# zju3dv/Mirror-NeRF

Hardware: AMD Instinct MI355X
Metric: rendered rays/sec (primary+reflected) (higher is better)
Workload: dtype f32 carried as hi/lo f16 pairs (f16 MFMA, f32 accumulate; max |diff| to the fp32 chain 3e-6)

## Files before the change

mirror_nerf_amd/csrc/mnrf_composite.inc:

```
struct CompMaps {
    float* weights;
    float* opacity; float* rgb_map; float* depth; float* mirror_mask;
    float* surf_normal; float* surf_normal_grad; float* normal_dif; float* x_surface;
    const float* rays;
    int white_back;
};

template <class Src>
__device__ __forceinline__ float composite_weight(const Src& src, int S, int s, bool in, int lane, float& carry, float& zv) {
    float alpha = 0.f;
    zv = 0.f;
    if (in) {
        zv = src.z(s);
        const float delta = s + 1 < S ? src.z(s + 1) - zv : 1e10f;
        float sv = src.sigma(s);
        if (src.has_noise()) sv = sv + src.noise(s);
        alpha = 1.f - expf(-delta * fmaxf(sv, 0.f));
    }
    const float t = in ? (1.f - alpha) + 1e-10f : 1.f;
    float incl = t;
#pragma unroll
    for (int o = 1; o < 64; o <<= 1) {
        const float up = __shfl_up(incl, o);
        if (lane >= o) incl *= up;
    }
    float excl = __shfl_up(incl, 1);
    if (lane == 0) excl = 1.f;
    const float w = alpha * (carry * excl);
    carry = carry * __shfl(incl, 63);
    return w;
}

template <class Src>
__device__ __forceinline__ float composite_mirror_value(const Src& src, int S, int lane, float* w_keep) {
    float carry = 1.f;
    float a_m = 0.f;
#pragma unroll
    for (int base = 0; base < S; base += 64) {
        const int s = base + lane;
        const bool in = s < S;
        float zv;
        const float w = composite_weight(src, S, s, in, lane, carry, zv);
        if (in) {
            if (w_keep) w_keep[s] = w;
            a_m += w * src.mirror(s);
        }
    }
    return wave_sum(a_m);
}

template <class Src>
__device__ __forceinline__ void composite_ray(const Src& src, int S, int lane, long long ray, const CompMaps& A) {
    float carry = 1.f;
    float a_op = 0.f, a_d = 0.f, a_m = 0.f, a_nd = 0.f;
    float a_c[3] = {0.f, 0.f, 0.f}, a_n[3] = {0.f, 0.f, 0.f}, a_g[3] = {0.f, 0.f, 0.f};
    for (int base = 0; base < S; base += 64) {
        const int s = base + lane;
        const bool in = s < S;
        float zv, w;
        if (src.has_w()) {
            zv = in ? src.z(s) : 0.f;
            w = in ? src.w(s) : 0.f;
        } else {
            w = composite_weight(src, S, s, in, lane, carry, zv);
        }
        if (in) {
            if (A.weights) A.weights[s] = w;
            a_op += w;
            a_d += w * zv;
            if (src.has_rgb()) { a_c[0] += w * src.rgb(s, 0); a_c[1] += w * src.rgb(s, 1); a_c[2] += w * src.rgb(s, 2); }
            if (src.has_mirror()) a_m += w * src.mirror(s);
            float pn[3] = {0.f, 0.f, 0.f}, gn[3] = {0.f, 0.f, 0.f};
            if (src.has_pn()) {
#pragma unroll
                for (int k = 0; k < 3; ++k) { pn[k] = src.pn(s, k); a_n[k] += pn[k] * w; }
            }
            if (src.has_gn()) {
#pragma unroll
                for (int k = 0; k < 3; ++k) { gn[k] = src.gn(s, k); a_g[k] += gn[k] * w; }
            }
            if (src.has_pn() && src.has_gn()) {
                const float d0 = gn[0] - pn[0], d1 = gn[1] - pn[1], d2 = gn[2] - pn[2];
                a_nd += w * (d0 * d0 + d1 * d1 + d2 * d2);
            }
        }
    }
    a_op = wave_sum(a_op);
    a_d = wave_sum(a_d);
    if (src.has_mirror()) a_m = wave_sum(a_m);
    if (src.has_pn() && src.has_gn()) a_nd = wave_sum(a_nd);
#pragma unroll
    for (int k = 0; k < 3; ++k) {
        if (src.has_rgb()) a_c[k] = wave_sum(a_c[k]);
        if (src.has_pn()) a_n[k] = wave_sum(a_n[k]);
        if (src.has_gn()) a_g[k] = wave_sum(a_g[k]);
    }
    if (lane == 0) {
        if (A.opacity) A.opacity[ray] = a_op;
        if (A.rgb_map) {
#pragma unroll
            for (int k = 0; k < 3; ++k) A.rgb_map[ray * 3 + k] = A.white_back ? a_c[k] + (1.f - a_op) : a_c[k];
        }
        if (A.depth) A.depth[ray] = a_d;
        if (A.mirror_mask) A.mirror_mask[ray] = a_m;
        if (A.surf_normal) { for (int k = 0; k < 3; ++k) A.surf_normal[ray * 3 + k] = a_n[k]; }
        if (A.surf_normal_grad) { for (int k = 0; k < 3; ++k) A.surf_normal_grad[ray * 3 + k] = a_g[k]; }
        if (A.normal_dif) A.normal_dif[ray] = a_nd;
        if (A.x_surface) {
            const float* r = A.rays + ray * 8;
            for (int k = 0; k < 3; ++k) A.x_surface[ray * 3 + k] = r[k] + r[3 + k] * a_d;
        }
    }
}
```

mirror_nerf_amd/csrc/mnrf_field_split.inc:

```
constexpr int CHUNK_BYTES = CHUNK_PAIRS * PAIR_BYTES;
constexpr int WAVES = 4;
constexpr int WG_THREADS = 64 * WAVES;
constexpr int WG_SAMPLES = WAVES * S * 16;
constexpr int PIECES = CHUNK_BYTES / TILE_BYTES / WAVES;
constexpr int U = 2;
constexpr int PF = S == 3 ? 2 : 4;
constexpr int NBUF = PF + U;
typedef unsigned u32x4 __attribute__((ext_vector_type(4)));
typedef unsigned u32x2 __attribute__((ext_vector_type(2)));
typedef _Float16 h2v __attribute__((ext_vector_type(2)));
struct StoreCtx {
    __amdgpu_buffer_rsrc_t rsrc;
    __amdgpu_buffer_rsrc_t rsrc_lo;
    char* base;
    int lane;
    int soff;
    h2v fac[S];
};
__device__ __forceinline__ __amdgpu_buffer_rsrc_t plane_rsrc(char* sample_block) {
    return __builtin_amdgcn_make_buffer_rsrc(sample_block, 0, 0x7fffffff, 0x00020000);
}
static_assert(CHUNK_PAIRS / U == PIECES, "one LDS-DMA piece per wave per unit");
constexpr int LDS_RING = RING_SLOTS * CHUNK_BYTES;
constexpr int LDS_BIAS = LDS_RING;
constexpr int LDS_MASK = LDS_BIAS + BIAS_FLOATS * 4;
constexpr int LDS_PARK = LDS_MASK;
constexpr int HEAD_PARK = 6;
constexpr int LDS_PARK_BYTES = S == 3 ? HEAD_PARK * S * WG_THREADS * 16 : 0;
static_assert(S != 3 || HEAD_PARK * S >= 2 * S * 2, "the encoding operands fit the same region");
constexpr int LDS_TILEQ = LDS_MASK + LDS_PARK_BYTES;
constexpr int LDS_BYTES = LDS_TILEQ + 16;
constexpr int LDS_BYTES_GRAD = LDS_MASK + 8 * S * WG_THREADS * 8;
static_assert(LDS_BYTES_GRAD <= 160 * 1024, "LDS budget");
constexpr int LDS_FUSE = LDS_BYTES;
constexpr int LDS_BYTES_FUSE = LDS_BYTES + 10 * WG_SAMPLES * 4;
static_assert(LDS_BYTES_FUSE <= 160 * 1024, "LDS budget");

#include "mnrf_field_split_common.inc"

__device__ __forceinline__ float wave_sum(float v) {
#pragma unroll
    for (int o = 32; o > 0; o >>= 1) v += __shfl_xor(v, o);
    return v;
}
#include "mnrf_composite.inc"
struct CompLdsSrc {
    const float* f;
    bool pn_on, mir_on;
    __device__ __forceinline__ bool has_w() const { return false; }
    __device__ __forceinline__ float w(int) const { return 0.f; }
    __device__ __forceinline__ bool has_noise() const { return false; }
    __device__ __forceinline__ bool has_rgb() const { return true; }
    __device__ __forceinline__ bool has_mirror() const { return mir_on; }
    __device__ __forceinline__ bool has_pn() const { return pn_on; }
    __device__ __forceinline__ bool has_gn() const { return false; }
    __device__ __forceinline__ float z(int s) const { return f[8 * WG_SAMPLES + s]; }
    __device__ __forceinline__ float sigma(int s) const { return f[s]; }
    __device__ __forceinline__ float noise(int) const { return 0.f; }
    __device__ __forceinline__ float rgb(int s, int k) const { return f[(1 + k) * WG_SAMPLES + s]; }
    __device__ __forceinline__ float mirror(int s) const { return f[7 * WG_SAMPLES + s]; }
    __device__ __forceinline__ float pn(int s, int k) const { return f[(4 + k) * WG_SAMPLES + s]; }
    __device__ __forceinline__ float gn(int, int) const { return 0.f; }
};
struct CompLdsSrcBlended : CompLdsSrc {
    bool colour;
    __device__ __forceinline__ bool has_rgb() const { return colour; }
    __device__ __forceinline__ bool has_w() const { return true; }
    __device__ __forceinline__ float w(int s) const { return f[9 * WG_SAMPLES + s]; }
};
struct CompLdsSrcRgbDepth : CompLdsSrc {
    __device__ __forceinline__ bool has_mirror() const { return false; }
    __device__ __forceinline__ bool has_pn() const { return false; }
};

__device__ __forceinline__ unsigned long long enc_out_of_range(const float (&x)[S][3]) {
    bool big = false;
#pragma unroll
    for (int s = 0; s < S; ++s) big |= !(fabsf(x[s][0]) < ENC_RANGE_LIMIT && fabsf(x[s][1]) < ENC_RANGE_LIMIT && fabsf(x[s][2]) < ENC_RANGE_LIMIT);
    return __builtin_amdgcn_ballot_w64(big);
}

template <int N>
__device__ __forceinline__ void split_b(const float (&x)[S][N], u32x4 (&hi)[S][N / 8], u32x4 (&lo)[S][N / 8],
                                        unsigned long long& sat, float limit = F16_MAX) {
    float tmax = 0.f;
#pragma unroll
    for (int s = 0; s < S; ++s)
#pragma unroll
        for (int T = 0; T < N / 8; ++T)
#pragma unroll
            for (int e = 0; e < 4; ++e) {
                unsigned h, l;
                split2(x[s][8 * T + 2 * e], x[s][8 * T + 2 * e + 1], h, l);
                sat_track<false>(tmax, x[s][8 * T + 2 * e], x[s][8 * T + 2 * e + 1]);
                hi[s][T][e] = h;
                lo[s][T][e] = l;
            }
    sat_flush(sat, tmax, limit);
}

__device__ __forceinline__ f32x4 mfma_f16(const u32x4& a, const u32x4& b, const f32x4& c) {
    return __builtin_amdgcn_mfma_f32_16x16x32_f16(__builtin_bit_cast(h8, a), __builtin_bit_cast(h8, b), c, 0, 0, 0);
}

__device__ __forceinline__ float relu_(float x) {
    const int i = __builtin_bit_cast(int, x);
    return __builtin_bit_cast(float, i > 0 ? i : 0);
}

constexpr int NTASKS = 16 * S;
template <int ACT, bool WANT_MASK>
__device__ __forceinline__ void conv_task(int q, const f32x4 (&pacc)[S][8], u32x4 (&oh)[S][8], u32x4 (&ol)[S][8],
                                          int t0, int half, uint64_t (&mk)[S], float& tmax) {
    const int trel = q / (4 * S), s = (q / 4) % S, nb = 2 * trel + ((q >> 1) & 1), rp = q & 1;
    const float a0 = pacc[s][nb][2 * rp], a1 = pacc[s][nb][2 * rp + 1];
    if (WANT_MASK) {
        mk[s] |= (uint64_t)(a0 > 0.f) << (4 * (8 * half + nb) + 2 * rp);
        mk[s] |= (uint64_t)(a1 > 0.f) << (4 * (8 * half + nb) + 2 * rp + 1);
    }
    const float v0 = ACT == 1 ? relu_(a0) : a0, v1 = ACT == 1 ? relu_(a1) : a1;
    unsigned h, l;
    split2(v0, v1, h, l);
    sat_track<ACT == 1>(tmax, v0, v1);
    oh[s][t0 + trel][2 * (nb & 1) + rp] = h;
    ol[s][t0 + trel][2 * (nb & 1) + rp] = l;
}

template <int NT, int NB, int NACC, int NTA, int JOB, bool WANT_MASK, int USTART, int TPU, int POS, int NPARK = 0, int STB = -1,
          int STN = 4, bool SSCALE = false, int JUMP_T = -1, long long JUMP = 0, bool SKIP = false>
__device__ __forceinline__ void gemm_part_impl(f32x4 (&acc)[S][NACC], const u32x4 (&bh)[S][NTA], const u32x4 (&bl)[S][NTA],
                                               Stream& st, int wave, int lane16, const f32x4 (&pacc)[S][8],
                                               u32x4 (&oh)[S][8], u32x4 (&ol)[S][8], int t0, int half, uint64_t (&mk)[S],
                                               const StoreCtx& sc = StoreCtx{}, bool jump_on = true) {
    static_assert(JUMP == 0 || (JUMP_T >= 0 && JUMP_T % U == 0 && JUMP_T < NT * NB && ((POS + JUMP_T) / U) % PIECES == PIECES - 1 && JUMP % CHUNK_BYTES == 0),
                  "the fill pointer jumps between two chunks");
    static_assert(STB < 0 || (S == 2 && NT * NB / U >= 8 * STN && STB + STN <= NTA), "8 store tasks per operand ride on the part's first units");
    static_assert(NT <= NTA, "B operand count");
    static_assert(JOB < 0 || NTASKS % TPU == 0, "tasks per unit");
    static_assert(JOB < 0 || USTART + NTASKS / TPU <= NT * NB / U, "the job fits the part");
    constexpr int NPAIRS = NT * NB;
    static_assert(NPAIRS % U == 0, "pairs come in units");
    const unsigned ring = (unsigned)(size_t)(__attribute__((address_space(3))) char*)smem + (unsigned)lane16;
    u32x4 ah[NBUF], al[NBUF];
    constexpr int START = POS % CHUNK_PAIRS;
    static_assert(POS % U == 0, "parts start on a unit");
    static_assert(NPAIRS >= PF, "a part is at least as long as the read-ahead");
    unsigned base = ring + st.rd_slot * CHUNK_BYTES;
#pragma unroll
    for (int i = 0; i < PF; ++i) {
        ah[i] = st.ch[i];
        al[i] = st.cl[i];
// ... 591 lines not shown
                    const float a0 = acc[s][0][R0], a1 = acc[s][0][R0 + 1], a2 = acc[s][0][R0 + 2];
                    const float inv = 1.f / sqrtf(fmaxf(a0 * a0 + a1 * a1 + a2 * a2, 1.1920928955078125e-07f));
                    float* o = A.pred_normal + (long long)sidx(s) * 3;
                    out_store(o, a0 * inv); out_store(o + 1, a1 * inv); out_store(o + 2, a2 * inv);
                    if (GRAD && A.save_inv)
                        A.save_inv[idx[s]] = (a0 * a0 + a1 * a1 + a2 * a2) > 1.1920928955078125e-07f ? inv : -inv;
                }
        }
    };
    {
        f32x4 acc[S][1];
        init_bias<1>(acc, BIAS_SIG, gq());
        gemm_part<8, 1, 960, HP>(acc, hh, hl, st, wave, lane16);
        if (FUSE) {
            if (gq() == 0) {
#pragma unroll
                for (int s = 0; s < S; ++s) fz[wave * (S * 16) + s * 16 + m15()] = acc[s][0][0];
            }
        } else if (A.sigma && g == 0) {
#pragma unroll
            for (int s = 0; s < S; ++s)
                if (sval(s)) out_store(A.sigma + sidx(s), acc[s][0][0]);
        }
        if constexpr (FOLD && !RGB_DEPTH) put_normal(acc, std::integral_constant<int, 1>{});
    }

    bool colour = true;
    if (!SIGMA_ONLY) {
        if constexpr (!FOLD) {
            u32x4 nh[S][4], nl[S][4];
            {
                f32x4 acc[S][8];
                init_bias<8>(acc, BIAS_NRM1, gq());
                gemm_part<8, 8, 968, HP, ST0>(acc, hh, hl, st, wave, lane16, at_h(7, 0));
                if (keep) save_acc<8, 0>(A.save_x + (long long)SEC_HN * A.B, 128, 0, acc, idx, valid, g, unused_bits);
                acc_to_b<8, 0, false>(nh, nl, acc, 0, tid, st.sat);
                if constexpr (S == 2) { if (pl) store_planes<4, 4>(sc, SEC_HN / 16, nh, nl); }
            }
            f32x4 acc[S][1];
            init_bias<1>(acc, BIAS_NRM2, gq());
            gemm_part<4, 1, 1032>(acc, nh, nl, st, wave, lane16);
            put_normal(acc, std::integral_constant<int, 0>{});
        }
        const auto mirror_head = [&]() {
            u32x4 mh[S][4], ml[S][4];
            {
                f32x4 acc[S][8];
                init_bias<8>(acc, BIAS_MIR1, gq());
                gemm_part<8, 8, BLENDED ? 968 : FOLD ? FOLD_POS_MIR1 : 1036, HP, ST4, 4, false, JT, JUMP_FROM_MIRB>(acc, hh, hl, st, wave, lane16, at_h(7, 4));
                if (keep) {
                    uint64_t bits[S];
                    save_acc<8, 2>(A.save_x + (long long)SEC_HM * A.B, 128, 0, acc, idx, valid, g, bits);
#pragma unroll
                    for (int s = 0; s < S; ++s) gmask[(9 * S + s) * WG_THREADS + tid] = bits[s];
                } else if (GRAD && pl) {
                    store_sign_mask<8>(acc, gmask + (9 * S) * WG_THREADS + tid);
                }
                acc_to_b<8, 2, false>(mh, ml, acc, 0, tid, st.sat);
                if constexpr (S == 2) { if (pl) store_planes<4, 4>(sc, SEC_HM / 16, mh, ml); }
            }
            f32x4 acc[S][1];
            init_bias<1>(acc, BIAS_MIR2, gq());
            gemm_part<4, 1, BLENDED ? 1032 : FOLD ? FOLD_POS_MIR2 : 1100>(acc, mh, ml, st, wave, lane16);
            if (FUSE) {
                if (gq() == 0) {
#pragma unroll
                    for (int s = 0; s < S; ++s) fz[7 * WG_SAMPLES + wave * (S * 16) + s * 16 + m15()] = sigmoidf_(acc[s][0][0]);
                }
            } else if (A.is_mirror && g == 0) {
#pragma unroll
                for (int s = 0; s < S; ++s)
                    if (sval(s)) out_store(A.is_mirror + sidx(s), sigmoidf_(acc[s][0][0]));
            }
        };
        if constexpr (!FOLD) mirror_head();
        if constexpr (BLENDED) {
            mirror_head();
            skip_pairs4<1036>(st, wave, lane16);
            asm volatile("s_waitcnt lgkmcnt(0)" ::: "memory");
            __builtin_amdgcn_s_barrier();
            asm volatile("" ::: "memory");
            int dl;
            asm volatile("v_mbcnt_lo_u32_b32 %0, -1, 0\n\tv_mbcnt_hi_u32_b32 %0, -1, %0" : "=v"(dl));
            const float mv = composite_mirror_value(CompLdsSrc{fz, false, true}, WG_SAMPLES, dl, wave == 0 ? fz + 9 * WG_SAMPLES : nullptr);
            colour = __builtin_amdgcn_readfirstlane((int)(mv < 0.5f)) != 0 || A.fuse == 4;
        }
        const auto view_operands = [&](u32x4 (&vh)[S][1], u32x4 (&vl)[S][1]) {
            float de[S][8];
            const int gv = gq();
            const int spr = opaque_spr();
#pragma unroll
            for (int s = 0; s < S; ++s) {
                const float* dp = A.dir_emb + (long long)(sidx(s) / spr) * A.dir_stride;
#pragma unroll
                for (int t = 0; t < 8; ++t) {
                    const int e = 16 * (t >> 2) + 4 * gv + (t & 3);
                    de[s][t] = e < ENC_DIR ? dp[e] : 0.f;
                }
            }
            if (keep) save_bform<8>(A.save_x + (long long)SEC_DIRE * A.B, 32, de, idx, valid, g);
            split_b<8>(de, vh, vl, st.sat);
            if constexpr (S == 2) { if (pl) store_planes<1, 1>(sc, SEC_DIRE / 16, vh, vl); }
        };
        if (colour) {
            u32x4 dh[S][4], dl[S][4];
            if constexpr (FOLD) {
                u32x4 vh[S][1], vl[S][1];
                view_operands(vh, vl);
                f32x4 acc[S][8];
                init_bias<8>(acc, BIAS_DIR, gq());
                gemm_part<8, 8, BLENDED ? 1040 : FOLD_POS_DIR, HP>(acc, hh, hl, st, wave, lane16);
                gemm_part<1, 8, BLENDED ? 1104 : FOLD_POS_VIEW>(acc, vh, vl, st, wave, lane16);
                acc_to_b<8, 1, false>(dh, dl, acc, 0, tid, st.sat);
            } else {
                u32x4 fh[S][8], fl[S][8];
                {
                    f32x4 acc[S][16];
                    init_bias<16>(acc, BIAS_FIN, gq());
                    gemm_part<8, 16, 1104, HP>(acc, hh, hl, st, wave, lane16);
                    if (keep) save_acc<16, 0>(A.save_x + (long long)SEC_FIN * A.B, 256, 0, acc, idx, valid, g, unused_bits);
                    acc_to_b<16, 0, false>(fh, fl, acc, 0, tid, st.sat);
                    if constexpr (S == 2) { if (pl) store_planes<8, 8>(sc, SEC_FIN / 16, fh, fl); }
                }
                u32x4 vh[S][1], vl[S][1];
                view_operands(vh, vl);
                f32x4 acc[S][8];
                init_bias<8>(acc, BIAS_DIR, gq());
                gemm_part<8, 8, 1232>(acc, fh, fl, st, wave, lane16);
                gemm_part<1, 8, 1296>(acc, vh, vl, st, wave, lane16);
                if (keep) {
                    uint64_t bits[S];
                    save_acc<8, 1>(A.save_x + (long long)SEC_HD * A.B, 128, 0, acc, idx, valid, g, bits);
#pragma unroll
                    for (int s = 0; s < S; ++s) gmask[(8 * S + s) * WG_THREADS + tid] = bits[s];
                } else if (GRAD && pl) {
                    store_sign_mask<8>(acc, gmask + (8 * S) * WG_THREADS + tid);
                }
                acc_to_b<8, 1, false>(dh, dl, acc, 0, tid, st.sat);
                if constexpr (S == 2) { if (pl) store_planes<4, 4>(sc, SEC_HD / 16, dh, dl); }
            }
            f32x4 acc[S][1];
            init_bias<1>(acc, BIAS_RGB, gq());
            gemm_part<4, 1, BLENDED ? 1112 : FOLD ? FOLD_POS_RGB : 1304>(acc, dh, dl, st, wave, lane16);
            if (FUSE) {
                if (gq() == 0) {
#pragma unroll
                    for (int s = 0; s < S; ++s) {
                        const int q = wave * (S * 16) + s * 16 + (int)m15();
                        fz[1 * WG_SAMPLES + q] = sigmoidf_(acc[s][0][0]);
                        fz[2 * WG_SAMPLES + q] = sigmoidf_(acc[s][0][1]);
                        fz[3 * WG_SAMPLES + q] = sigmoidf_(acc[s][0][2]);
                    }
                }
            } else if (A.rgb && g == 0) {
#pragma unroll
                for (int s = 0; s < S; ++s)
                    if (sval(s)) {
                        float* o = A.rgb + (long long)sidx(s) * 3;
                        out_store(o, sigmoidf_(acc[s][0][0]));
                        out_store(o + 1, sigmoidf_(acc[s][0][1]));
                        out_store(o + 2, sigmoidf_(acc[s][0][2]));
                    }
            }
        }
        if constexpr (FOLD && !RGB_DEPTH && !BLENDED) mirror_head();
    }

// ... 12 lines not shown
                    for (int r = 0; r < 4; ++r) gr[s][4 * nb + r] = v[r];
            }
        }
        float genc[S][16];
#pragma unroll
        for (int s = 0; s < S; ++s)
#pragma unroll
            for (int t = 0; t < 16; ++t) genc[s][t] = 0.f;

#pragma unroll 1
        for (int layer = 7; layer >= 0; --layer) {
            u32x4 gh[S][8], gl[S][8];
#pragma unroll
            for (int s = 0; s < S; ++s) {
                const uint64_t mk = ((const uint64_t*)(smem + LDS_MASK))[(layer * S + s) * WG_THREADS + tid];
#pragma unroll
                for (int t = 0; t < 64; ++t) gr[s][t] = ((mk >> t) & 1ull) ? gr[s][t] : 0.f;
            }
            split_b<64>(gr, gh, gl, st.sat);
            if (layer == 4 || layer == 0) {
                f32x4 acc[S][4];
                zero_acc<4>(acc);
                gemm_part<8, 4, 0>(acc, gh, gl, st, wave, lane16);
#pragma unroll
                for (int s = 0; s < S; ++s)
#pragma unroll
                    for (int nb = 0; nb < 4; ++nb)
#pragma unroll
                        for (int r = 0; r < 4; ++r) genc[s][4 * nb + r] += acc[s][nb][r];
            }
            if (layer != 0) {
                f32x4 acc[S][16];
                zero_acc<16>(acc);
                gemm_part<8, 16, 0>(acc, gh, gl, st, wave, lane16);
#pragma unroll
                for (int s = 0; s < S; ++s)
#pragma unroll
                    for (int nb = 0; nb < 16; ++nb)
#pragma unroll
                        for (int r = 0; r < 4; ++r) gr[s][4 * nb + r] = acc[s][nb][r];
            }
        }
        float x[S][3];
        fetch_positions(x);
#pragma unroll
        for (int s = 0; s < S; ++s) {
            float d0 = 0.f, d1 = 0.f, d2 = 0.f;
#pragma unroll
            for (int pp = 0; pp < 8; ++pp) {
                const int P = 8 * g + pp;
                const int f = P / 3;
                const int a = P - 3 * f;
                const float gs = genc[s][2 * pp], gc = genc[s][2 * pp + 1];
                if (P < 30) {
                    const float xa = a == 0 ? x[s][0] : (a == 1 ? x[s][1] : x[s][2]);
                    float sn, cs;
                    fast_sincos(ldexpf(xa, f), sn, cs);
                    const float c = ldexpf(gs * cs - gc * sn, f);
                    d0 += a == 0 ? c : 0.f;
                    d1 += a == 1 ? c : 0.f;
                    d2 += a == 2 ? c : 0.f;
                } else if (P == 30) {
                    d0 += gs;
                    d1 += gc;
                } else {
                    d2 += gs;
                }
            }
            d0 += __shfl_xor(d0, 16); d1 += __shfl_xor(d1, 16); d2 += __shfl_xor(d2, 16);
            d0 += __shfl_xor(d0, 32); d1 += __shfl_xor(d1, 32); d2 += __shfl_xor(d2, 32);
            if (A.normal && g == 0 && valid[s]) {
                const float n0 = -d0, n1 = -d1, n2 = -d2;
                const float sq = n0 * n0 + n1 * n1 + n2 * n2;
                const float inv = 1.f / sqrtf(fmaxf(sq, 1.1920928955078125e-07f));
                float* o = A.normal + (long long)idx[s] * 3;
                o[0] = n0 * inv; o[1] = n1 * inv; o[2] = n2 * inv;
                if (A.save_invj) A.save_invj[idx[s]] = sq > 1.1920928955078125e-07f ? inv : -inv;
            }
        }
    }
    sat_all |= st.sat;
    enc_all |= enc_range;
    if (FUSE) {
        __syncthreads();
        if (wave == 0) {
            const long long ray = tile;
            int cl;
            asm volatile("v_mbcnt_lo_u32_b32 %0, -1, 0\n\tv_mbcnt_hi_u32_b32 %0, -1, %0" : "=v"(cl));
            if constexpr (RGB_DEPTH) {
                const CompMaps out{A.f_weights ? A.f_weights + ray * WG_SAMPLES : nullptr, A.f_opacity, A.f_rgb_map, A.f_depth, nullptr,
                                   nullptr, nullptr, nullptr, A.f_x_surface, A.rays, A.white_back};
                composite_ray(CompLdsSrcRgbDepth{fz, false, false}, WG_SAMPLES, cl, ray, out);
            } else if constexpr (BLENDED) {
                const CompLdsSrcBlended src{{fz, A.f_surf_normal != nullptr, A.f_mirror_mask != nullptr}, colour};
                const CompMaps out{A.f_weights ? A.f_weights + ray * WG_SAMPLES : nullptr, A.f_opacity, colour ? A.f_rgb_map : nullptr, A.f_depth,
                                   A.f_mirror_mask, A.f_surf_normal, nullptr, nullptr, A.f_x_surface, A.rays, A.white_back};
                composite_ray(src, WG_SAMPLES, cl, ray, out);
                if (!colour && A.f_rgb_map && cl < 3) A.f_rgb_map[ray * 3 + cl] = 0.f;
            } else {
                const CompLdsSrc src{fz, A.f_surf_normal != nullptr, A.f_mirror_mask != nullptr};
                const CompMaps out{A.f_weights ? A.f_weights + ray * WG_SAMPLES : nullptr, A.f_opacity, A.f_rgb_map, A.f_depth, A.f_mirror_mask,
                                   A.f_surf_normal, nullptr, nullptr, A.f_x_surface, A.rays, A.white_back};
                composite_ray(src, WG_SAMPLES, cl, ray, out);
            }
        }
    }
    if (!queued) break;
    close_stream();
    __syncthreads();
    tile = __builtin_amdgcn_readfirstlane(((volatile int*)(smem + LDS_TILEQ))[round & 1]);
    ++round;
    if (tile >= A.n_tiles) break;
    }
    guard_report(A.packed, sat_all, enc_all, MNRF_GUARD_IN_FORWARD);
    close_stream();
    int last_lane;
    asm volatile("v_mbcnt_lo_u32_b32 %0, -1, 0\n\tv_mbcnt_hi_u32_b32 %0, -1, %0" : "=v"(last_lane));
    if (queued && wave == 0 && last_lane == 0) {
        if (atomicAdd(A.tile_queue + 1, 1) == (int)gridDim.x - 1) {
            atomicExch(A.tile_queue, 0);
            atomicExch(A.tile_queue + 1, 0);
        }
    }
}

template <bool SIGMA_ONLY, bool GRAD, bool PLANES = false, bool FUSE = false>
__global__ __launch_bounds__(WG_THREADS, MIN_WAVES_PER_SIMD) void field_split_kernel(FieldArgs A) {
    field_split_body<SIGMA_ONLY, GRAD, PLANES, FUSE, false>(A);
}
template <bool ON = true>
__global__ __launch_bounds__(WG_THREADS, MIN_WAVES_PER_SIMD) void field_split_kernel_rgb_depth(FieldArgs A) {
    field_split_body<false, false, false, ON, ON>(A);
}

template <bool ON = true>
__global__ __launch_bounds__(WG_THREADS, MIN_WAVES_PER_SIMD) void field_split_kernel_blended(FieldArgs A) {
    field_split_body<false, false, false, ON, false, ON>(A);
}

template <bool UNUSED = false>
inline int launch(const FieldArgs& A, bool sigma_only, bool grad, hipStream_t s) {
    const long long blocks64 = (A.B + WG_SAMPLES - 1) / WG_SAMPLES;
    if (blocks64 > 0x7fffffff || A.B > 0x7fffffffLL) return -1;
    dim3 grid((unsigned)blocks64);
    const dim3 block(WG_THREADS);
    if (S == 3 && A.tile_queue) {
        if (A.n_tiles != (int)blocks64 || A.resident < 1 || A.resident > A.n_tiles) return -1;
        grid = dim3((unsigned)A.resident);
    }
    if (sigma_only && !grad) hipLaunchKernelGGL((field_split_kernel<true, false>), grid, block, LDS_BYTES, s, A);
    else if (!sigma_only && !grad && S == 3 && A.fuse == 2) {
        if constexpr (S == 3) hipLaunchKernelGGL((field_split_kernel_rgb_depth<>), grid, block, LDS_BYTES_FUSE, s, A);
    } else if (!sigma_only && !grad && S == 3 && A.fuse >= 3) {
        if constexpr (S == 3) hipLaunchKernelGGL((field_split_kernel_blended<>), grid, block, LDS_BYTES_FUSE, s, A);
    } else if (!sigma_only && !grad && S == 3 && A.fuse)
        hipLaunchKernelGGL((field_split_kernel<false, false, false, S == 3>), grid, block, LDS_BYTES_FUSE, s, A);
    else if (!sigma_only && !grad) hipLaunchKernelGGL((field_split_kernel<false, false>), grid, block, LDS_BYTES, s, A);
#ifndef MNRF_SPLIT_NO_GRAD
    else if (sigma_only && grad) hipLaunchKernelGGL((field_split_kernel<true, true>), grid, block, LDS_BYTES_GRAD, s, A);
    else if (S == 2 && A.save_planes) hipLaunchKernelGGL((field_split_kernel<false, true, S == 2>), grid, block, LDS_BYTES_GRAD, s, A);
    else hipLaunchKernelGGL((field_split_kernel<false, true>), grid, block, LDS_BYTES_GRAD, s, A);
#else
    else return -1;
#endif
    return 0;
}
```

mirror_nerf_amd/csrc/mnrf_render.hip:

```cpp
#include <hip/hip_runtime.h>
#include <stdint.h>
#include <stdio.h>
#include <string.h>

#include "../../include/mnrf.h"
#include "mnrf_error.h"
#include "mnrf_fill.h"
#include "mnrf_rays.h"

static thread_local char g_err[512] = "";

int mnrf_fail(int code, const char* msg) {
    snprintf(g_err, sizeof(g_err), "%s", msg);
    return code;
}

int mnrf_check_launch(const char* where) {
    hipError_t e = hipGetLastError();
    if (e != hipSuccess) {
        snprintf(g_err, sizeof(g_err), "%s: %s", where, hipGetErrorString(e));
        return MNRF_ERR_LAUNCH;
    }
    return MNRF_OK;
}

extern "C" const char* mnrf_last_error(void) { return g_err; }
extern "C" int mnrf_version(void) { return 1; }

namespace {

constexpr float EPS32 = 1.1920928955078125e-07f;

__device__ __forceinline__ long long live_rows(long long cap, const int* __restrict__ n_live) {
    if (!n_live) return cap;
    const long long v = *n_live;
    return v < 0 ? 0 : (v < cap ? v : cap);
}

__device__ __forceinline__ float wave_sum(float v) {
#pragma unroll
    for (int o = 32; o > 0; o >>= 1) v += __shfl_xor(v, o);
    return v;
}
#include "mnrf_composite.inc"

__global__ void embed_kernel(const float* __restrict__ x, long long n, int c, int n_freqs, float* __restrict__ out,
                             const int* __restrict__ n_live) {
    const long long i = (long long)blockIdx.x * blockDim.x + threadIdx.x;
    if (i >= live_rows(n, n_live) * c) return;
    const long long row = i / c;
    const int ch = (int)(i % c);
    const int ld = c * (2 * n_freqs + 1);
    const float v = x[i];
    float* o = out + row * ld;
    o[ch] = v;
    for (int f = 0; f < n_freqs; ++f) {
        float s, co;
        sincosf(ldexpf(v, f), &s, &co);
        o[c * (1 + 2 * f) + ch] = s;
        o[c * (2 + 2 * f) + ch] = co;
    }
}

__global__ void sample_coarse_kernel(const float* __restrict__ rays, long long n_rays, const float* __restrict__ z_steps,
                                     int ns, int use_disp, float perturb, const float* __restrict__ prand,
                                     float* __restrict__ z_out, const int* __restrict__ n_live) {
    const long long i = (long long)blockIdx.x * blockDim.x + threadIdx.x;
    if (i >= live_rows(n_rays, n_live) * ns) return;
    const long long r = i / ns;
    const int s = (int)(i % ns);
    const float near = rays[r * 8 + 6], far = rays[r * 8 + 7];
    auto zat = [&](int k) -> float {
        const float t = z_steps[k];
        if (!use_disp) return near * (1.f - t) + far * t;
        return 1.f / (1.f / near * (1.f - t) + 1.f / far * t);
    };
    float z = zat(s);
    if (perturb > 0.f) {
        const float lower = s == 0 ? z : 0.5f * (zat(s - 1) + z);
        const float upper = s == ns - 1 ? z : 0.5f * (z + zat(s + 1));
        z = lower + (upper - lower) * (perturb * prand[i]);
    }
    z_out[i] = z;
}

struct CompArgs {
    const float* rays; long long n_rays; int S;
    const float* sigma; const float* z; const float* noise; const float* rgb; const float* is_mirror;
    const float* pred_normal; const float* normal; int white_back;
    float* weights; float* opacity; float* rgb_map; float* depth; float* mirror_mask;
    float* surf_normal; float* surf_normal_grad; float* normal_dif; float* x_surface;
    const int* n_live;
};

struct CompGlobalSrc {
    const CompArgs& A;
    long long ray;
    __device__ __forceinline__ bool has_w() const { return false; }
    __device__ __forceinline__ float w(int) const { return 0.f; }
    __device__ __forceinline__ bool has_noise() const { return A.noise != nullptr; }
    __device__ __forceinline__ bool has_rgb() const { return A.rgb != nullptr; }
    __device__ __forceinline__ bool has_mirror() const { return A.is_mirror != nullptr; }
    __device__ __forceinline__ bool has_pn() const { return A.pred_normal != nullptr; }
    __device__ __forceinline__ bool has_gn() const { return A.normal != nullptr; }
    __device__ __forceinline__ float z(int s) const { return A.z[ray * A.S + s]; }
    __device__ __forceinline__ float sigma(int s) const { return A.sigma[ray * A.S + s]; }
    __device__ __forceinline__ float noise(int s) const { return A.noise[ray * A.S + s]; }
    __device__ __forceinline__ float rgb(int s, int k) const { return A.rgb[(ray * A.S + s) * 3 + k]; }
    __device__ __forceinline__ float mirror(int s) const { return A.is_mirror[ray * A.S + s]; }
    __device__ __forceinline__ float pn(int s, int k) const { return A.pred_normal[(ray * A.S + s) * 3 + k]; }
    __device__ __forceinline__ float gn(int s, int k) const { return A.normal[(ray * A.S + s) * 3 + k]; }
};

__global__ __launch_bounds__(256) void composite_kernel(CompArgs A) {
    const int lane = threadIdx.x & 63;
    const long long ray = (long long)blockIdx.x * 4 + (threadIdx.x >> 6);
    if (ray >= live_rows(A.n_rays, A.n_live)) return;
    const CompGlobalSrc src{A, ray};
    const CompMaps out{A.weights ? A.weights + ray * A.S : nullptr, A.opacity, A.rgb_map, A.depth, A.mirror_mask, A.surf_normal,
                       A.surf_normal_grad, A.normal_dif, A.x_surface, A.rays, A.white_back};
    composite_ray(src, A.S, lane, ray, out);
}


struct CompBwdArgs {
    const float* rays; long long n_rays; int S;
    const float* sigma; const float* z; const float* noise; const float* rgb; const float* is_mirror;
    const float* pred_normal; const float* normal; int white_back;
    const float* depth;
    const float* g_w; const float* g_op; const float* g_rgb; const float* g_depth; const float* g_mask;
    const float* g_sn; const float* g_sng; const float* g_nd; const float* g_xs;
    float* d_sigma; float* d_rgb; float* d_mirror; float* d_pn; float* d_n; float* d_rays;
    int detach;
    const float* keep_mirror;
    const int* n_live;
};
constexpr int CB_MAXB = 4;

__global__ __launch_bounds__(256) void composite_backward_kernel(CompBwdArgs A) {
    const int lane = threadIdx.x & 63;
    const long long ray = (long long)blockIdx.x * 4 + (threadIdx.x >> 6);
    if (ray >= live_rows(A.n_rays, A.n_live)) return;
    const int S = A.S;
    const float* r8 = A.rays ? A.rays + ray * 8 : nullptr;
    float gop = A.g_op ? A.g_op[ray] : 0.f;
    float gc[3] = {0.f, 0.f, 0.f}, gsn[3] = {0.f, 0.f, 0.f}, gsg[3] = {0.f, 0.f, 0.f}, gxs[3] = {0.f, 0.f, 0.f};
    if (A.g_rgb) { for (int k = 0; k < 3; ++k) gc[k] = A.g_rgb[ray * 3 + k]; }
    if (A.g_sn) { for (int k = 0; k < 3; ++k) gsn[k] = A.g_sn[ray * 3 + k]; }
    if (A.g_sng) { for (int k = 0; k < 3; ++k) gsg[k] = A.g_sng[ray * 3 + k]; }
    if (A.g_xs) { for (int k = 0; k < 3; ++k) gxs[k] = A.g_xs[ray * 3 + k]; }
    float gd = A.g_depth ? A.g_depth[ray] : 0.f;
    const float gm = A.g_mask ? A.g_mask[ray] : 0.f;
    const float gnd = A.g_nd ? A.g_nd[ray] : 0.f;
    const bool w_mask = !(A.detach & MNRF_DETACH_W_MASK) && !(A.keep_mirror && A.keep_mirror[ray] == 0.f);
    const bool w_nrm = !(A.detach & MNRF_DETACH_W_NORMAL);
    const float gm_w = w_mask ? gm : 0.f;
    const float gnd_w = w_nrm ? gnd : 0.f;
    float gsn_w[3], gsg_w[3];
    for (int k = 0; k < 3; ++k) { gsn_w[k] = w_nrm ? gsn[k] : 0.f; gsg_w[k] = w_nrm ? gsg[k] : 0.f; }
    if (A.g_xs && r8) gd += gxs[0] * r8[3] + gxs[1] * r8[4] + gxs[2] * r8[5];
    if (A.white_back) gop -= gc[0] + gc[1] + gc[2];
    if (A.d_rays && lane == 0) {
        float* o = A.d_rays + ray * 8;
        const float dep = A.depth ? A.depth[ray] : 0.f;
        for (int k = 0; k < 3; ++k) { o[k] = gxs[k]; o[3 + k] = gxs[k] * dep; }
        o[6] = 0.f; o[7] = 0.f;
    }
    float Tn[CB_MAXB], Gw[CB_MAXB], Gv[CB_MAXB], tv[CB_MAXB], dads[CB_MAXB];
    float carry = 1.f;
#pragma unroll
    for (int blk = 0; blk < CB_MAXB; ++blk) {
        Tn[blk] = 0.f; Gw[blk] = 0.f; Gv[blk] = 0.f; tv[blk] = 1.f; dads[blk] = 0.f;
        if (blk * 64 >= S) continue;
        const int s = blk * 64 + lane;
        const bool in = s < S;
        const long long i1 = ray * S + s, i3 = i1 * 3;
        float alpha = 0.f, G = 0.f, delta = 0.f, sv = 0.f, ex = 1.f;
        float pn[3] = {0.f, 0.f, 0.f}, gn[3] = {0.f, 0.f, 0.f};
        if (in) {
            const float zv = A.z[i1];
            delta = s + 1 < S ? A.z[i1 + 1] - zv : 1e10f;
            sv = A.sigma[i1];
// ... 983 lines not shown
```

mirror_nerf_amd/recursion.py:

```python
import ctypes
import os
from collections import defaultdict
import weakref
from types import SimpleNamespace

import torch
from torch import nn

from . import _lib
from .mirror_nerf import Embedding, MirrorNeRF
from .dnerf import render_rays_dnerf
from .rendering import render_rays

RAY_FORWARD_OFFSET = 0.1
BLENDED_BREAK_EVEN = 0.37
_MIRROR_FRACTION = weakref.WeakKeyDictionary()
JITTER_RAYS = 262144

PLACE_MIRROR_PRESETS = {
    "plane_x": (
        ("livingroom", dict(position=0.0, normal=(-1.0, 0.0, 0.0), rect=(-1.0, 1.0, -0.5, 0.5))),
        ("washroom", dict(position=-1.0, normal=(1.0, 0.0, 0.0), rect=(-1.0, 1.0, -1.0, 0.75))),
        ("office", dict(position=1.0, normal=(1.0, 0.0, 0.0), rect=(-1.0, 1.0, -1.0, 0.75))),
        (None, dict(position=-1.0, normal=(1.0, 0.0, 0.0), rect=(-1.0, 1.0, -0.5, 0.5))),
    ),
    "plane_y": (
        ("washroom", dict(position=1.3, normal=(0.0, -1.0, 0.0), rect=(-1.0, 1.0, -1.0, 1.0))),
        ("livingroom", dict(position=1.65, normal=(0.0, -1.0, 0.0), rect=(-0.3, 1.5, -0.5, 1.0))),
        ("office", dict(position=0.0, normal=(0.0, -1.0, 0.0), rect=(-1.0, 1.0, -0.5, 0.5))),
        (None, dict(position=1.0, normal=(0.0, -1.0, 0.0), rect=(-1.0, 1.0, -0.5, 0.5))),
    ),
}
SUBSTITUTION_PRESETS = (
    ("office", dict(rotation=None, scale=1.0, translation=(0.0, 1.0, 0.0))),
    ("market", dict(rotation=((0.0, 1.0, 0.0), (-1.0, 0.0, 0.0), (0.0, 0.0, 1.0)), scale=1.0,
                    translation=(0.0, 0.0, 0.0))),
    (None, dict(rotation=None, scale=1.0, translation=(0.0, 0.0, 0.0))),
)
OBJECT_PRESETS = (
    ("livingroom", dict(pose_align=None, scale=2.0, translation=(0.0, 0.0, 0.0))),
    ("washroom", dict(pose_align=None, scale=2.0, translation=(-0.5, -0.5, 0.0))),
    ("office", dict(pose_align=None, scale=2.0, translation=(0.0, 3.0, 0.5))),
    (None, dict(pose_align=None, scale=1.0, translation=(0.0, 0.0, 0.0))),
)


def _preset(table, root_dir):
    for key, value in table:
        if key is None or key in (root_dir or ""):
            return dict(value)
    raise AssertionError("preset tables end with a default entry")


def resolve_new_mirror(args, new_mirror=None):
    if new_mirror is not None:
        nm = dict(new_mirror)
        missing = {"axis", "position", "normal", "rect"} - set(nm)
        if missing:
            raise ValueError(f"new_mirror needs the keys axis, position, normal, rect (missing: {sorted(missing)})")
        if nm["axis"] not in ("x", "y"):
            raise ValueError(f"new_mirror axis must be 'x' or 'y', not {nm['axis']!r}")
        if len(nm["normal"]) != 3 or len(nm["rect"]) != 4:
            raise ValueError("new_mirror normal has 3 entries and rect 4 (u0, u1, w0, w1)")
        return dict(axis=nm["axis"], position=float(nm["position"]), normal=tuple(float(v) for v in nm["normal"]),
                    rect=tuple(float(v) for v in nm["rect"]))
    plane_pos = getattr(args, "plane_pos", "plane_x")
    if plane_pos not in PLACE_MIRROR_PRESETS:
        raise ValueError(f"args.plane_pos must be 'plane_x' or 'plane_y', not {plane_pos!r}")
    p = _preset(PLACE_MIRROR_PRESETS[plane_pos], getattr(args, "root_dir", ""))
    return dict(axis=plane_pos[-1], **p)


def resolve_substitution(args):
    return _preset(SUBSTITUTION_PRESETS, getattr(args, "root_dir", ""))


def resolve_new_object(args, new_object=None):
    if new_object is not None:
        cfg = dict(new_object)
        missing = {"pose_align", "scale", "translation"} - set(cfg)
        if missing:
            raise ValueError(f"new_object needs the keys pose_align, scale, translation (missing: {sorted(missing)})")
    else:
        cfg = _preset(OBJECT_PRESETS, getattr(args, "root_dir", ""))
    if len(cfg["translation"]) != 3:
        raise ValueError("new_object translation has 3 entries")
    scale = float(cfg["scale"])
    if not scale > 0.0:
        raise ValueError(f"new_object scale must be positive, not {cfg['scale']!r}")
    pose, pose_scale0 = None, 1.0
    if cfg["pose_align"] is not None:
        m = torch.as_tensor(cfg["pose_align"], dtype=torch.float32)
        if tuple(m.shape) not in ((3, 4), (4, 4)):
            raise ValueError(f"new_object pose_align must be None, 3x4 or 4x4, not {tuple(m.shape)}")
        pose = tuple(float(v) for v in m[:3, :4].reshape(-1))
        pose_scale0 = float(torch.norm(m[:3, 0]))
        if not pose_scale0 > 0.0:
            raise ValueError("new_object pose_align: the first column of its 3x3 is zero")
# ... 694 lines not shown
```

Measured before the change: 1.985 million.

## Split fused per-ray compositing across all four waves of the workgroup

```diff
diff --git a/mirror_nerf_amd/csrc/mnrf_composite.inc b/mirror_nerf_amd/csrc/mnrf_composite.inc
--- a/mirror_nerf_amd/csrc/mnrf_composite.inc
+++ b/mirror_nerf_amd/csrc/mnrf_composite.inc
@@ -7,8 +7,9 @@
 };
 
 template <class Src>
-__device__ __forceinline__ float composite_weight(const Src& src, int S, int s, bool in, int lane, float& carry, float& zv) {
-    float alpha = 0.f;
+__device__ __forceinline__ void composite_block_scan(const Src& src, int S, int s, bool in, int lane, float& alpha, float& zv, float& excl,
+                                                     float& total) {
+    alpha = 0.f;
     zv = 0.f;
     if (in) {
         zv = src.z(s);
@@ -24,29 +25,18 @@
         const float up = __shfl_up(incl, o);
         if (lane >= o) incl *= up;
     }
-    float excl = __shfl_up(incl, 1);
+    excl = __shfl_up(incl, 1);
     if (lane == 0) excl = 1.f;
+    total = __shfl(incl, 63);
+}
+
+template <class Src>
+__device__ __forceinline__ float composite_weight(const Src& src, int S, int s, bool in, int lane, float& carry, float& zv) {
+    float alpha, excl, total;
+    composite_block_scan(src, S, s, in, lane, alpha, zv, excl, total);
     const float w = alpha * (carry * excl);
-    carry = carry * __shfl(incl, 63);
+    carry = carry * total;
     return w;
-}
-
-template <class Src>
-__device__ __forceinline__ float composite_mirror_value(const Src& src, int S, int lane, float* w_keep) {
-    float carry = 1.f;
-    float a_m = 0.f;
-#pragma unroll
-    for (int base = 0; base < S; base += 64) {
-        const int s = base + lane;
-        const bool in = s < S;
-        float zv;
-        const float w = composite_weight(src, S, s, in, lane, carry, zv);
-        if (in) {
-            if (w_keep) w_keep[s] = w;
-            a_m += w * src.mirror(s);
-        }
-    }
-    return wave_sum(a_m);
 }
 
 template <class Src>
@@ -57,13 +47,8 @@
     for (int base = 0; base < S; base += 64) {
         const int s = base + lane;
         const bool in = s < S;
-        float zv, w;
-        if (src.has_w()) {
-            zv = in ? src.z(s) : 0.f;
-            w = in ? src.w(s) : 0.f;
-        } else {
-            w = composite_weight(src, S, s, in, lane, carry, zv);
-        }
+        float zv;
+        const float w = composite_weight(src, S, s, in, lane, carry, zv);
         if (in) {
             if (A.weights) A.weights[s] = w;
             a_op += w;
@@ -112,3 +97,113 @@
         }
     }
 }
+
+constexpr int COMP_WG_SAMPLES = 192;
+
+__device__ __forceinline__ void composite_wg_barrier() {
+    asm volatile("s_waitcnt lgkmcnt(0)" ::: "memory");
+    __builtin_amdgcn_s_barrier();
+    asm volatile("" ::: "memory");
+}
+
+template <class Src>
+__device__ __forceinline__ void composite_weights_wg(const Src& src, int wave, int lane, float* totals, float* w_row, float* w_out) {
+    const int s = wave * 64 + lane;
+    float alpha = 0.f, zv = 0.f, excl = 1.f, total = 1.f;
+    if (wave < 3) {
+        composite_block_scan(src, COMP_WG_SAMPLES, s, true, lane, alpha, zv, excl, total);
+        if (lane == 0) totals[wave] = total;
+    }
+    composite_wg_barrier();
+    if (wave < 3) {
+        float carry = 1.f;
+        if (wave >= 1) carry = carry * totals[0];
+        if (wave >= 2) carry = carry * totals[1];
+        const float w = alpha * (carry * excl);
+        w_row[s] = w;
+        if (w_out) w_out[s] = w;
+    }
+    composite_wg_barrier();
+}
+
+template <class X>
+__device__ __forceinline__ float composite_wg_sum(const float* w_row, int lane, const X& x) {
+    float a = 0.f;
+#pragma unroll
+    for (int base = 0; base < COMP_WG_SAMPLES; base += 64) a += w_row[base + lane] * x(base + lane);
+    return wave_sum(a);
+}
+__device__ __forceinline__ float composite_wg_opacity(const float* w_row, int lane) {
+    float a = 0.f;
+#pragma unroll
+    for (int base = 0; base < COMP_WG_SAMPLES; base += 64) a += w_row[base + lane];
+    return wave_sum(a);
+}
+
+template <class Src>
+__device__ __forceinline__ void composite_maps_wg(const Src& src, int wave, int lane, const float* w_row, long long ray, const CompMaps& A) {
+    if (A.weights && wave < 3) A.weights[wave * 64 + lane] = w_row[wave * 64 + lane];
+    if (wave == 0) {
+        const float a_op = composite_wg_opacity(w_row, lane);
+        const float a_d = composite_wg_sum(w_row, lane, [&](int s) { return src.z(s); });
+        if (lane == 0) {
+            if (A.opacity) A.opacity[ray] = a_op;
+            if (A.depth) A.depth[ray] = a_d;
+            if (A.x_surface) {
+                const float* r = A.rays + ray * 8;
+                for (int k = 0; k < 3; ++k) A.x_surface[ray * 3 + k] = r[k] + r[3 + k] * a_d;
+            }
+        }
+    } else if (wave == 1) {
+        if (A.rgb_map) {
+            float a_c[3] = {0.f, 0.f, 0.f};
+            if (src.has_rgb()) {
+#pragma unroll
+                for (int k = 0; k < 3; ++k) a_c[k] = composite_wg_sum(w_row, lane, [&](int s) { return src.rgb(s, k); });
+            }
+            float a_op = 0.f;
+            if (A.white_back) a_op = composite_wg_opacity(w_row, lane);
+            if (lane == 0) {
+#pragma unroll
+                for (int k = 0; k < 3; ++k) A.rgb_map[ray * 3 + k] = A.white_back ? a_c[k] + (1.f - a_op) : a_c[k];
+            }
+        }
+    } else if (wave == 2) {
+        if (src.has_pn() || src.has_gn()) {
+            float a_n[3] = {0.f, 0.f, 0.f}, a_g[3] = {0.f, 0.f, 0.f}, a_nd = 0.f;
+#pragma unroll
+            for (int k = 0; k < 3; ++k) {
+                if (src.has_pn()) a_n[k] = composite_wg_sum(w_row, lane, [&](int s) { return src.pn(s, k); });
+                if (src.has_gn()) a_g[k] = composite_wg_sum(w_row, lane, [&](int s) { return src.gn(s, k); });
+            }
+            if (src.has_pn() && src.has_gn())
+                a_nd = composite_wg_sum(w_row, lane, [&](int s) {
+                    const float d0 = src.gn(s, 0) - src.pn(s, 0), d1 = src.gn(s, 1) - src.pn(s, 1), d2 = src.gn(s, 2) - src.pn(s, 2);
+                    return d0 * d0 + d1 * d1 + d2 * d2;
+                });
+            if (lane == 0) {
+                if (A.surf_normal) { for (int k = 0; k < 3; ++k) A.surf_normal[ray * 3 + k] = a_n[k]; }
+                if (A.surf_normal_grad) { for (int k = 0; k < 3; ++k) A.surf_normal_grad[ray * 3 + k] = a_g[k]; }
+                if (A.normal_dif) A.normal_dif[ray] = a_nd;
+            }
+        } else if (lane == 0) {
+            if (A.surf_normal) { for (int k = 0; k < 3; ++k) A.surf_normal[ray * 3 + k] = 0.f; }
+            if (A.surf_normal_grad) { for (int k = 0; k < 3; ++k) A.surf_normal_grad[ray * 3 + k] = 0.f; }
+            if (A.normal_dif) A.normal_dif[ray] = 0.f;
+        }
+    } else {
+        if (A.mirror_mask) {
+            float a_m = 0.f;
+            if (src.has_mirror()) a_m = composite_wg_sum(w_row, lane, [&](int s) { return src.mirror(s); });
+            if (lane == 0) A.mirror_mask[ray] = a_m;
+        }
+    }
+}
+
+template <class Src>
+__device__ __forceinline__ void composite_ray_wg(const Src& src, int wave, int lane, float* totals, float* w_row, long long ray, const CompMaps& A) {
+    composite_weights_wg(src, wave, lane, totals, w_row, A.weights);
+    CompMaps B = A;
+    B.weights = nullptr;
+    composite_maps_wg(src, wave, lane, w_row, ray, B);
+}
diff --git a/mirror_nerf_amd/csrc/mnrf_field_split.inc b/mirror_nerf_amd/csrc/mnrf_field_split.inc
--- a/mirror_nerf_amd/csrc/mnrf_field_split.inc
+++ b/mirror_nerf_amd/csrc/mnrf_field_split.inc
@@ -33,7 +33,7 @@
 constexpr int LDS_BYTES_GRAD = LDS_MASK + 8 * S * WG_THREADS * 8;
 static_assert(LDS_BYTES_GRAD <= 160 * 1024, "LDS budget");
 constexpr int LDS_FUSE = LDS_BYTES;
-constexpr int LDS_BYTES_FUSE = LDS_BYTES + 10 * WG_SAMPLES * 4;
+constexpr int LDS_BYTES_FUSE = LDS_BYTES + 10 * WG_SAMPLES * 4 + 16;
 static_assert(LDS_BYTES_FUSE <= 160 * 1024, "LDS budget");
 
 #include "mnrf_field_split_common.inc"
@@ -47,8 +47,6 @@
 struct CompLdsSrc {
     const float* f;
     bool pn_on, mir_on;
-    __device__ __forceinline__ bool has_w() const { return false; }
-    __device__ __forceinline__ float w(int) const { return 0.f; }
     __device__ __forceinline__ bool has_noise() const { return false; }
     __device__ __forceinline__ bool has_rgb() const { return true; }
     __device__ __forceinline__ bool has_mirror() const { return mir_on; }
@@ -65,8 +63,6 @@
 struct CompLdsSrcBlended : CompLdsSrc {
     bool colour;
     __device__ __forceinline__ bool has_rgb() const { return colour; }
-    __device__ __forceinline__ bool has_w() const { return true; }
-    __device__ __forceinline__ float w(int s) const { return f[9 * WG_SAMPLES + s]; }
 };
 struct CompLdsSrcRgbDepth : CompLdsSrc {
     __device__ __forceinline__ bool has_mirror() const { return false; }
@@ -824,7 +820,8 @@
             asm volatile("" ::: "memory");
             int dl;
             asm volatile("v_mbcnt_lo_u32_b32 %0, -1, 0\n\tv_mbcnt_hi_u32_b32 %0, -1, %0" : "=v"(dl));
-            const float mv = composite_mirror_value(CompLdsSrc{fz, false, true}, WG_SAMPLES, dl, wave == 0 ? fz + 9 * WG_SAMPLES : nullptr);
+            composite_weights_wg(CompLdsSrc{fz, false, true}, wave, dl, fz + 10 * WG_SAMPLES, fz + 9 * WG_SAMPLES, nullptr);
+            const float mv = composite_wg_sum(fz + 9 * WG_SAMPLES, dl, [&](int q) { return fz[7 * WG_SAMPLES + q]; });
             colour = __builtin_amdgcn_readfirstlane((int)(mv < 0.5f)) != 0 || A.fuse == 4;
         }
         const auto view_operands = [&](u32x4 (&vh)[S][1], u32x4 (&vl)[S][1]) {
@@ -1003,27 +1000,28 @@
     sat_all |= st.sat;
     enc_all |= enc_range;
     if (FUSE) {
+        static_assert(!FUSE || WG_SAMPLES == COMP_WG_SAMPLES, "the workgroup form composites 3 x 64 samples");
         __syncthreads();
-        if (wave == 0) {
-            const long long ray = tile;
-            int cl;
-            asm volatile("v_mbcnt_lo_u32_b32 %0, -1, 0\n\tv_mbcnt_hi_u32_b32 %0, -1, %0" : "=v"(cl));
-            if constexpr (RGB_DEPTH) {
-                const CompMaps out{A.f_weights ? A.f_weights + ray * WG_SAMPLES : nullptr, A.f_opacity, A.f_rgb_map, A.f_depth, nullptr,
-                                   nullptr, nullptr, nullptr, A.f_x_surface, A.rays, A.white_back};
-                composite_ray(CompLdsSrcRgbDepth{fz, false, false}, WG_SAMPLES, cl, ray, out);
-            } else if constexpr (BLENDED) {
-                const CompLdsSrcBlended src{{fz, A.f_surf_normal != nullptr, A.f_mirror_mask != nullptr}, colour};
-                const CompMaps out{A.f_weights ? A.f_weights + ray * WG_SAMPLES : nullptr, A.f_opacity, colour ? A.f_rgb_map : nullptr, A.f_depth,
-                                   A.f_mirror_mask, A.f_surf_normal, nullptr, nullptr, A.f_x_surface, A.rays, A.white_back};
-                composite_ray(src, WG_SAMPLES, cl, ray, out);
-                if (!colour && A.f_rgb_map && cl < 3) A.f_rgb_map[ray * 3 + cl] = 0.f;
-            } else {
-                const CompLdsSrc src{fz, A.f_surf_normal != nullptr, A.f_mirror_mask != nullptr};
-                const CompMaps out{A.f_weights ? A.f_weights + ray * WG_SAMPLES : nullptr, A.f_opacity, A.f_rgb_map, A.f_depth, A.f_mirror_mask,
-                                   A.f_surf_normal, nullptr, nullptr, A.f_x_surface, A.rays, A.white_back};
-                composite_ray(src, WG_SAMPLES, cl, ray, out);
-            }
+        const long long ray = tile;
+        int cl;
+        asm volatile("v_mbcnt_lo_u32_b32 %0, -1, 0\n\tv_mbcnt_hi_u32_b32 %0, -1, %0" : "=v"(cl));
+        float* const w_row = fz + 9 * WG_SAMPLES;
+        float* const totals = fz + 10 * WG_SAMPLES;
+        if constexpr (RGB_DEPTH) {
+            const CompMaps out{A.f_weights ? A.f_weights + ray * WG_SAMPLES : nullptr, A.f_opacity, A.f_rgb_map, A.f_depth, nullptr,
+                               nullptr, nullptr, nullptr, A.f_x_surface, A.rays, A.white_back};
+            composite_ray_wg(CompLdsSrcRgbDepth{fz, false, false}, wave, cl, totals, w_row, ray, out);
+        } else if constexpr (BLENDED) {
+            const CompLdsSrcBlended src{{fz, A.f_surf_normal != nullptr, A.f_mirror_mask != nullptr}, colour};
+            const CompMaps out{A.f_weights ? A.f_weights + ray * WG_SAMPLES : nullptr, A.f_opacity, colour ? A.f_rgb_map : nullptr, A.f_depth,
+                               A.f_mirror_mask, A.f_surf_normal, nullptr, nullptr, A.f_x_surface, A.rays, A.white_back};
+            composite_maps_wg(src, wave, cl, w_row, ray, out);
+            if (!colour && A.f_rgb_map && wave == 1 && cl < 3) A.f_rgb_map[ray * 3 + cl] = 0.f;
+        } else {
+            const CompLdsSrc src{fz, A.f_surf_normal != nullptr, A.f_mirror_mask != nullptr};
+            const CompMaps out{A.f_weights ? A.f_weights + ray * WG_SAMPLES : nullptr, A.f_opacity, A.f_rgb_map, A.f_depth, A.f_mirror_mask,
+                               A.f_surf_normal, nullptr, nullptr, A.f_x_surface, A.rays, A.white_back};
+            composite_ray_wg(src, wave, cl, totals, w_row, ray, out);
         }
     }
     if (!queued) break;
diff --git a/mirror_nerf_amd/csrc/mnrf_render.hip b/mirror_nerf_amd/csrc/mnrf_render.hip
--- a/mirror_nerf_amd/csrc/mnrf_render.hip
+++ b/mirror_nerf_amd/csrc/mnrf_render.hip
@@ -96,8 +96,6 @@
 struct CompGlobalSrc {
     const CompArgs& A;
     long long ray;
-    __device__ __forceinline__ bool has_w() const { return false; }
-    __device__ __forceinline__ float w(int) const { return 0.f; }
     __device__ __forceinline__ bool has_noise() const { return A.noise != nullptr; }
     __device__ __forceinline__ bool has_rgb() const { return A.rgb != nullptr; }
     __device__ __forceinline__ bool has_mirror() const { return A.is_mirror != nullptr; }
diff --git a/mirror_nerf_amd/recursion.py b/mirror_nerf_amd/recursion.py
--- a/mirror_nerf_amd/recursion.py
+++ b/mirror_nerf_amd/recursion.py
@@ -13,7 +13,7 @@
 from .rendering import render_rays
 
 RAY_FORWARD_OFFSET = 0.1
-BLENDED_BREAK_EVEN = 0.37
+BLENDED_BREAK_EVEN = 0.18
 _MIRROR_FRACTION = weakref.WeakKeyDictionary()
 JITTER_RAYS = 262144
 
```

After: 1.993 million (median of 6 runs). No clear change (+0.4%).
